# bowen-upenn/scene_graph_commonsense

Measured on AMD Instinct MI355X. Metric: ordered object-pairs/sec (relation head fwd+bwd), batch=8, N=64, higher is better.
Workload: dtype f16 fwd / bf16 bwd (f32 accumulate, f32 master weights); 1 GPU; VG PredCLS synthetic, 8 images x 64 objects per GPU = 32256 ordered pairs per GPU per step, from the raw minibatch; parallelism=dp1

## Files before the change

scene_graph_commonsense_amd/csrc/gemm_nt.h:

```cpp
#pragma once
#include "common.h"
#include <type_traits>

enum { AMODE_PLAIN = 0, AMODE_CONV = 1, AMODE_CONV_GATHER = 2 };
enum { EPI_STORE = 0, EPI_BIAS_TANH = 1, EPI_BIAS_RELU = 2, EPI_POOL = 3, EPI_FC2 = 4, EPI_RELUMASK = 5, EPI_STORE_F32 = 6,
       EPI_STORE_F32T = 7 };

struct NtParams {
    const u16* A; const u16* B; void* C;
    int M, N, K;
    long lda, ldb, ldc;
    int lgS, Cin;
    const float* bias;
    const u16* mask_src;
    const float* lsub; const float* lobj; const int* sub_idx; const int* obj_idx;
    unsigned char* argmax;
    u16* C2;
    float scale;
    unsigned drop_seed; int drop_enable;
    int tiles_m, tiles_n;
    int epi_lds;
    int halo_walk;
    int patch_aligned;
    const u16* Apool; const unsigned char* Acode;
    const int* gather; const int* gather_n;
    const int* dest;
    const int* wm_goff;
    float* raw; int raw_first;
    const int* tile_group; long group_stride;
    u16* Cx; int x_first;
    long seg_stride; int seg_bpad, seg_split;
};

template <int ELEM>
__device__ __forceinline__ f32x16 mfma32(s16x8 a, s16x8 b, f32x16 c) {
    if constexpr (ELEM == ELEM_F16) {
        return __builtin_amdgcn_mfma_f32_32x32x16_f16(__builtin_bit_cast(f16x8, a), __builtin_bit_cast(f16x8, b), c, 0, 0, 0);
    } else {
        return __builtin_amdgcn_mfma_f32_32x32x16_bf16(__builtin_bit_cast(bf16x8, a), __builtin_bit_cast(bf16x8, b), c, 0, 0, 0);
    }
}

__device__ __forceinline__ long conv_row_base(int m, int lgS, int Cin) {
    const int S = 1 << lgS;
    const int img = m >> (2 * lgS);
    const int ml = m & (S * S - 1);
    const int W = ml >> 2, q = ml & 3;
    const int py = W >> (lgS - 1), px = W & ((S >> 1) - 1);
    const int y = 2 * py + (q >> 1), x = 2 * px + (q & 1);
    return ((long)(img * (S + 2) + y) * (S + 2) + x) * Cin;
}

template <int ELEM, int EPI, int TM, int TN, bool GATHER = false>
__device__ __forceinline__ void nt_epilogue(const NtParams& p, f32x16 (&acc)[TM][TN], int m0, int n0, int wr, int wc, int lane, int m_limit = -1) {
    const int M = GATHER ? m_limit : p.M;
    const int h = lane >> 5, cl = lane & 31;
#pragma unroll
    for (int i = 0; i < TM; ++i) {
#pragma unroll
        for (int j = 0; j < TN; ++j) {
            const int col = n0 + wc * TN * 32 + j * 32 + cl;
            const int rbase = m0 + wr * TM * 32 + i * 32;
            const float bias = p.bias ? p.bias[col] : 0.f;
            if constexpr (EPI == EPI_POOL) {
                u16* out = reinterpret_cast<u16*>(p.C);
#pragma unroll
                for (int w = 0; w < 4; ++w) {
                    float v = acc[i][j][4 * w];
                    int am = 0;
#pragma unroll
                    for (int q = 1; q < 4; ++q) {
                        const float t = acc[i][j][4 * w + q];
                        if (t > v) { v = t; am = q; }
                    }
                    v += bias;
                    const int prow = (rbase >> 2) + 2 * w + h;
                    if (prow * 4 < M) {
                        long arow = prow, yrow = prow;
                        if constexpr (GATHER) {
                            arow = p.gather[prow]; yrow = p.dest ? p.dest[prow] : arow;
                            if (p.raw && prow >= p.raw_first) {
#pragma unroll
                                for (int q = 0; q < 4; ++q) p.raw[((long)(prow - p.raw_first) * 4 + q) * p.ldc + col] = acc[i][j][4 * w + q];
                            }
                        }
                        else if (p.wm_goff) yrow = p.wm_goff[prow & 63] + (prow >> 6);
                        if (!(v > 0.f)) { v = 0.f; am = 4; }
                        out[yrow * p.ldc + col] = to_elem<ELEM>(v);
                        if (p.C2) p.C2[yrow * p.ldc + col] = f32_to_bf16_bits(v);
                        if (p.argmax) p.argmax[arow * p.ldc + col] = (unsigned char)am;
                    }
                }
            } else {
#pragma unroll
                for (int r = 0; r < 16; ++r) {
                    const int row = rbase + (r & 3) + 8 * (r >> 2) + 4 * h;
                    if (row >= M) continue;
                    float v = acc[i][j][r];
                    long o = (long)row * p.ldc + col;
                    if constexpr (GATHER && EPI == EPI_STORE)
                        o = ((long)p.gather[row >> 2] * 4 + (row & 3)) * p.ldc + col;
                    if constexpr (EPI == EPI_STORE) {
                        reinterpret_cast<u16*>(p.C)[o] = to_elem<ELEM>(v + bias);
                    } else if constexpr (EPI == EPI_STORE_F32) {
                        reinterpret_cast<float*>(p.C)[o] = v + bias;
                    } else if constexpr (EPI == EPI_BIAS_TANH) {
                        reinterpret_cast<u16*>(p.C)[o] = to_elem<ELEM>(tanhf(v + bias));
                    } else if constexpr (EPI == EPI_BIAS_RELU) {
                        v = fmaxf(v + bias, 0.f);
                        if (p.drop_enable) v = dropout_keep(p.drop_seed, (uint32_t)(row * p.N + col)) ? v * p.scale : 0.f;
                        reinterpret_cast<u16*>(p.C)[o] = to_elem<ELEM>(v);
                    } else if constexpr (EPI == EPI_FC2) {
                        v += bias + p.lsub[(long)p.sub_idx[row] * p.N + col] + p.lobj[(long)p.obj_idx[row] * p.N + col];
                        v = fmaxf(v, 0.f);
                        if (p.drop_enable) v = dropout_keep(p.drop_seed, (uint32_t)(row * p.N + col)) ? v * p.scale : 0.f;
                        reinterpret_cast<float*>(p.C)[o] = v;
                    } else if constexpr (EPI == EPI_RELUMASK) {
                        const float f = from_elem<ELEM_F16>(p.mask_src[o]);
                        reinterpret_cast<u16*>(p.C)[o] = to_elem<ELEM>(f > 0.f ? v * p.scale : 0.f);
                    }
                }
            }
        }
    }
}

__device__ __forceinline__ void nt_epilogue_f32t(const NtParams& p, f32x16 (&acc)[4][2], int m0, int n0, int wr, int wc, int lane) {
    const int h = lane >> 5, cl = lane & 31;
    float* out = reinterpret_cast<float*>(p.C);
    if (!out) return;
    const int g_first = p.Cx ? p.wm_goff[p.tile_group[m0 >> 8]] + p.x_first : 0;
#pragma unroll
    for (int i = 0; i < 4; ++i) {
        const int row = m0 + wr * 128 + i * 32 + cl;
        if (row >= p.M) continue;
        const bool xrow = p.Cx && row >= g_first;
#pragma unroll
        for (int j = 0; j < 2; ++j) {
#pragma unroll
            for (int rq = 0; rq < 4; ++rq) {
                const int col = n0 + wc * 64 + j * 32 + 8 * rq + 4 * h;
                f32x4 v = {acc[i][j][4 * rq], acc[i][j][4 * rq + 1], acc[i][j][4 * rq + 2], acc[i][j][4 * rq + 3]};
                if (p.bias) {
                    const f32x4 b = *reinterpret_cast<const f32x4*>(p.bias + col);
                    v += b;
                }
                if (xrow) {
                    uint2 hv;
                    hv.x = (unsigned)f32_to_f16_bits(v[0]) | ((unsigned)f32_to_f16_bits(v[1]) << 16);
                    hv.y = (unsigned)f32_to_f16_bits(v[2]) | ((unsigned)f32_to_f16_bits(v[3]) << 16);
                    *reinterpret_cast<uint2*>(p.Cx + (long)row * p.N + col) = hv;
                    continue;
                }
                f32x4* dst = reinterpret_cast<f32x4*>(out + (long)row * p.ldc + col);
                *dst = v;
            }
        }
    }
}

__device__ __forceinline__ void supertile_map(int id, int tiles_m, int tiles_n, int& tm, int& tn) {
    constexpr int GS = 16;
    const int a = id / (GS * tiles_n);
    const int hm = min(GS, tiles_m - a * GS);
    const int id2 = id - a * GS * tiles_n;
    const int sn = (tiles_n + GS - 1) / GS;
    const int b = min(id2 / (hm * GS), sn - 1);
    const int id3 = id2 - b * hm * GS;
    const int wn = min(GS, tiles_n - b * GS);
    tm = a * GS + id3 / wn;
    tn = b * GS + id3 % wn;
}

__device__ __forceinline__ void supertile_map_g(int id, int tiles_m, int tiles_n, int GM, int GN, int& tm, int& tn) {
    const int a = id / (GM * tiles_n);
    const int hm = min(GM, tiles_m - a * GM);
    const int id2 = id - a * GM * tiles_n;
    const int sn = (tiles_n + GN - 1) / GN;
    const int b = min(id2 / (hm * GN), sn - 1);
    const int id3 = id2 - b * hm * GN;
    const int wn = min(GN, tiles_n - b * GN);
    tm = a * GM + id3 / wn;
    tn = b * GN + id3 % wn;
}

constexpr int EPI_LDS_PITCH = 128;
constexpr int EPI_LDS_BYTES = 8 * 128 * EPI_LDS_PITCH;
template <int ELEM, bool MASK = false>
__device__ __forceinline__ void nt_epilogue_store16(const NtParams& p, f32x16 (&acc)[4][2], int m0, int n0, int wr, int wc, int lane,
                                                    int wid, char* smem) {
    __syncthreads();
    char* reg = smem + wid * (128 * EPI_LDS_PITCH);
    const int h = lane >> 5, cl = lane & 31;
    const bool odd = cl & 1;
#pragma unroll
    for (int i = 0; i < 4; ++i) {
#pragma unroll
        for (int j = 0; j < 2; ++j) {
            const int col = n0 + wc * 64 + j * 32 + cl;
            const float bias = p.bias ? p.bias[col] : 0.f;
#pragma unroll
            for (int rp = 0; rp < 8; ++rp) {
                float v0 = acc[i][j][2 * rp] + bias, v1 = acc[i][j][2 * rp + 1] + bias;
                if constexpr (MASK) { v0 *= p.scale; v1 *= p.scale; }
                const float recv = __shfl_xor(odd ? v0 : v1, 1);
                const int r0 = ((2 * rp) & 3) + 8 * ((2 * rp) >> 2) + 4 * h;
                const float flo = odd ? recv : v0, fhi = odd ? v1 : recv;
                unsigned packed;
                if constexpr (ELEM == ELEM_BF16) packed = f32x2_to_bf16x2_bits(flo, fhi);
                else packed = (unsigned)to_elem<ELEM>(flo) | ((unsigned)to_elem<ELEM>(fhi) << 16);
                const int row = i * 32 + r0 + (odd ? 1 : 0);
                *reinterpret_cast<unsigned*>(reg + row * EPI_LDS_PITCH + (((j * 32 + (cl & ~1)) * 2) ^ ((row & 1) << 6))) = packed;
            }
        }
    }
    __builtin_amdgcn_wave_barrier();
    u16* out = reinterpret_cast<u16*>(p.C);
    const int c8 = lane & 7, rsub = lane >> 3;
#pragma unroll
    for (int it = 0; it < 16; ++it) {
        const int rowl = it * 8 + rsub;
        uint4 v = *reinterpret_cast<const uint4*>(reg + rowl * EPI_LDS_PITCH + ((c8 * 16) ^ ((rowl & 1) << 6)));
        const int row = m0 + wr * 128 + rowl;
        if (row < p.M) {
            const long o = (long)row * p.ldc + n0 + wc * 64 + c8 * 8;
            if constexpr (MASK) {
                const uint4 f = *reinterpret_cast<const uint4*>(p.mask_src + o);
                const u16* fh = reinterpret_cast<const u16*>(&f);
                u16* vh = reinterpret_cast<u16*>(&v);
#pragma unroll
                for (int k = 0; k < 8; ++k)
                    if (!(from_elem<ELEM_F16>(fh[k]) > 0.f)) vh[k] = 0;
            }
            *reinterpret_cast<uint4*>(out + o) = v;
        }
    }
}

template <int ELEM, int AMODE, int EPI, int WR, int WC, int TM, int TN>
__global__ __launch_bounds__(WR * WC * 64, 2) void gemm_nt_kernel(const NtParams p) {
    extern __shared__ __attribute__((aligned(16))) char smem[];
    constexpr int NW = WR * WC;
    constexpr int BM = WR * TM * 32, BN = WC * TN * 32;
    constexpr int A_BYTES = BM * 128, B_BYTES = BN * 128, BUF_BYTES = A_BYTES + B_BYTES;
    constexpr int AI = BM / (8 * NW), BI = BN / (8 * NW);
// ... 29 lines not shown
    const int Wp = (1 << p.lgS) + 2;

    auto stage = [&](int buf, int kt) {
        long aoff;
        if constexpr (AMODE != AMODE_PLAIN) {
            const int cc = kt / 9, tap = kt - cc * 9;
            const int ky = tap / 3, kx = tap - 3 * ky;
            aoff = (long)(ky * Wp + kx) * p.Cin + (cc << 6);
        } else {
            aoff = (long)kt << 6;
        }
        const long boff = (long)kt << 6;
        char* abase = smem + buf * BUF_BYTES + wid * (AI * 1024);
        char* bbase = smem + buf * BUF_BYTES + A_BYTES + wid * (BI * 1024);
#pragma unroll
        for (int i = 0; i < AI; ++i)
            __builtin_amdgcn_global_load_lds(GLB_PTR(a_ptr[i] + aoff), LDS_PTR(abase + i * 1024), 16, 0, 0);
#pragma unroll
        for (int i = 0; i < BI; ++i)
            __builtin_amdgcn_global_load_lds(GLB_PTR(b_ptr[i] + boff), LDS_PTR(bbase + i * 1024), 16, 0, 0);
    };

    const int wr = wid / WC, wc = wid % WC;
    const int kh = lane >> 5;
    int a_off[TM], a_sw[TM], b_off[TN], b_sw[TN];
#pragma unroll
    for (int i = 0; i < TM; ++i) {
        const int ra = wr * TM * 32 + i * 32 + (lane & 31);
        a_off[i] = ra * 128; a_sw[i] = (ra >> 1) & 7;
    }
#pragma unroll
    for (int i = 0; i < TN; ++i) {
        const int rb = wc * TN * 32 + i * 32 + (lane & 31);
        b_off[i] = rb * 128; b_sw[i] = (rb >> 1) & 7;
    }
    f32x16 acc[TM][TN];
#pragma unroll
    for (int i = 0; i < TM; ++i)
#pragma unroll
        for (int j = 0; j < TN; ++j)
#pragma unroll
            for (int r = 0; r < 16; ++r) acc[i][j][r] = 0.f;

    const int nk = p.K >> 6;
    stage(0, 0);
    for (int kt = 0; kt < nk; ++kt) {
        asm volatile("s_waitcnt vmcnt(0)" ::: "memory");
        __syncthreads();
        if (kt + 1 < nk) stage((kt + 1) & 1, kt + 1);
        const char* ab = smem + (kt & 1) * BUF_BYTES;
        const char* bb = ab + A_BYTES;
#pragma unroll
        for (int ks = 0; ks < 4; ++ks) {
            const int c = ks * 2 + kh;
            s16x8 af[TM], bf[TN];
#pragma unroll
            for (int i = 0; i < TM; ++i) af[i] = *reinterpret_cast<const s16x8*>(ab + a_off[i] + ((c ^ a_sw[i]) << 4));
#pragma unroll
            for (int i = 0; i < TN; ++i) bf[i] = *reinterpret_cast<const s16x8*>(bb + b_off[i] + ((c ^ b_sw[i]) << 4));
#pragma unroll
            for (int i = 0; i < TM; ++i)
#pragma unroll
                for (int j = 0; j < TN; ++j) acc[i][j] = mfma32<ELEM>(af[i], bf[j], acc[i][j]);
        }
    }

    if constexpr (EPI == EPI_STORE && TM == 4 && TN == 2 && WR * WC == 8) {
        if (p.epi_lds) { nt_epilogue_store16<ELEM>(p, acc, m0, n0, wr, wc, lane, wid, smem); return; }
    }
    if constexpr (AMODE == AMODE_CONV_GATHER) nt_epilogue<ELEM, EPI, TM, TN, true>(p, acc, m0, n0, wr, wc, lane, Mlim);
    else nt_epilogue<ELEM, EPI, TM, TN>(p, acc, m0, n0, wr, wc, lane);
}

template <int ELEM, int AMODE, int EPI, int WR, int WC, int TM, int TN>
static int launch_gemm_nt_cfg(NtParams p, hipStream_t stream) {
    constexpr int BM = WR * TM * 32, BN = WC * TN * 32;
    constexpr int LDS0 = 2 * (BM + BN) * 128;
    constexpr int LDS = (EPI == EPI_STORE && TM == 4 && TN == 2 && WR * WC == 8 && LDS0 < EPI_LDS_BYTES) ? EPI_LDS_BYTES : LDS0;
    p.tiles_m = (p.M + BM - 1) / BM;
    p.tiles_n = p.N / BN;
    auto kern = gemm_nt_kernel<ELEM, AMODE, EPI, WR, WC, TM, TN>;
    (void)hipFuncSetAttribute(reinterpret_cast<const void*>(kern), hipFuncAttributeMaxDynamicSharedMemorySize, LDS);
    SGC_LAUNCH(kern, dim3((unsigned)(p.tiles_m * p.tiles_n)), dim3(WR * WC * 64), LDS, stream, p);
    SGC_CHECK_LAUNCH();
    return SGC_OK;
}
// ... 22 lines not shown
```

scene_graph_commonsense_amd/csrc/gemm_nt_pp.h:

```cpp
#pragma once

#define SGC_WAIT_VM(n) asm volatile("s_waitcnt vmcnt(" #n ")" ::: "memory")
#define SGC_WAIT_LGKM0() asm volatile("s_waitcnt lgkmcnt(0)" ::: "memory")
#define SGC_PP_BARRIER()                                       \
    do {                                                       \
        __builtin_amdgcn_sched_barrier(0);                     \
        __builtin_amdgcn_s_barrier();                          \
        __builtin_amdgcn_sched_barrier(0);                     \
    } while (0)

__device__ __forceinline__ void buf_load_lds16(const void* base, int voff, int soff, void* lds) {
    const __amdgpu_buffer_rsrc_t r = __builtin_amdgcn_make_buffer_rsrc(const_cast<void*>(base), 0, 0x7fffffff, 0x00020000);
    __builtin_amdgcn_raw_ptr_buffer_load_lds(r, LDS_PTR(lds), 16, voff, soff, 0, 0);
}

__device__ __forceinline__ void xcd_patch_map(int id, int tiles_m, int tiles_n, int& tm, int& tn, int gm = 4, int gn = 8) {
    const int nb = tiles_m * tiles_n, q = nb >> 3, r = nb & 7, x = id & 7;
    const int lin = (x < r ? x * (q + 1) : r * (q + 1) + (x - r) * q) + (id >> 3);
    supertile_map_g(lin, tiles_m, tiles_n, gm, gn, tm, tn);
}

__host__ __device__ __forceinline__ int xcd_patch_gn(int tiles_n) { return tiles_n >= 8 ? 8 : (tiles_n >= 4 ? 4 : (tiles_n >= 2 ? 2 : 1)); }
static inline int xcd_patch_grid(int tiles_m, int tiles_n) {
    const int gn = xcd_patch_gn(tiles_n), gm = 32 / gn;
    const int npatch = ((tiles_m + gm - 1) / gm) * ((tiles_n + gn - 1) / gn);
    return ((npatch + 7) / 8) * 8 * 32;
}
__device__ __forceinline__ bool xcd_patch_map_aligned(int id, int tiles_m, int tiles_n, int& tm, int& tn) {
    const int gn = xcd_patch_gn(tiles_n), gm = 32 / gn;
    const int sn = (tiles_n + gn - 1) / gn, npatch = ((tiles_m + gm - 1) / gm) * sn;
    const int x = id & 7, j = id >> 3;
    const int patch = (j >> 5) * 8 + x, w = j & 31;
    if (patch >= npatch) return false;
    const int a = patch / sn, b = patch - a * sn;
    const int wn = min(gn, tiles_n - b * gn);
    tm = a * gm + w / wn;
    tn = b * gn + w % wn;
    return tm < tiles_m && w < gm * wn;
}

template <int ELEM, bool GATHER>
__device__ __forceinline__ void nt_epilogue_pool16(const NtParams& p, f32x16 (&acc)[4][2], int m0, int n0, int wr, int wc, int lane,
                                                   int wid, char* smem, int m_limit);
template <int ELEM, int EPI, int ACG = 0, int SEG = 0>
__global__ __launch_bounds__(512, 2) void gemm_nt_pp_kernel(const NtParams p) {
    extern __shared__ __attribute__((aligned(16))) char smem[];
    constexpr int HT = 16384;
    const int tid = threadIdx.x, lane = tid & 63;
    const int wid = __builtin_amdgcn_readfirstlane(tid >> 6);
    const int wr = wid >> 2, wc = wid & 3;
    int tm, tn;
    if constexpr (SEG) {
        xcd_patch_map(blockIdx.x, p.tiles_m, p.tiles_n, tm, tn, 16, 2);
    } else if (p.patch_aligned) {
        if (!xcd_patch_map_aligned(blockIdx.x, p.tiles_m, p.tiles_n, tm, tn)) return;
    } else {
        xcd_patch_map(blockIdx.x, p.tiles_m, p.tiles_n, tm, tn);
    }
    const int m0 = tm * 256;
    int n0 = tn * 256, n_tile = tn, Kloc = p.K, seg_py = 0, seg_px = 0, seg_ny = 1, seg_nx = 1, seg_c0 = 0;
    long ldb = p.ldb, b_off = 0;
    if constexpr (SEG) {
        const int slot = tn >> 1;
        int pp = 0, part = 0;
        if (p.seg_split) {
// ... 55 lines not shown
        char* base = smem + (((t & 1) << 2) + kind) * HT + wid * 2048;
        const u16* g = (kind == 0 || kind == 3) ? a_blk : b_blk;
        int soff = t << 7;
        if constexpr (ACG) {
            if (kind == 0 || kind == 3) {
                const int cc = t / 9, tap = t - cc * 9;
                const int ky = tap / 3, kx = tap - 3 * ky;
                soff = ((ky * SP + kx) * p.Cin + (cc << 6)) * 2;
            }
        }
        if constexpr (SEG) {
            if (kind == 0 || kind == 3) {
                const int c = seg_c0 + (t >> 4);
                const int cy = seg_nx == 2 ? (c >> 1) : c, cx = seg_nx == 2 ? (c & 1) : 0;
                const int qy = seg_ny == 1 ? (seg_py == 3) : cy, qx = seg_nx == 1 ? (seg_px == 3) : cx;
                g = a_blk + (long)(qy * 2 + qx) * p.seg_stride;
                soff = (t & 15) << 7;
            }
        }
        buf_load_lds16(g, voff[kind][0], soff, base);
        buf_load_lds16(g, voff[kind][1], soff, base + 1024);
    };

    const int l31 = lane & 31, kh = lane >> 5, sw = (l31 >> 1) & 7;
    int ko[4];
#pragma unroll
    for (int ks = 0; ks < 4; ++ks) ko[ks] = ((ks * 2 + kh) ^ sw) << 4;
    const int a_rd = (wr * 64 + l31) * 128, b_rd = (wc * 32 + l31) * 128;
    s16x8 af[2][4], bf[2][4];
    auto read_a = [&](int h, int par) __attribute__((always_inline)) {
        const char* base = smem + ((par << 2) + (h ? 3 : 0)) * HT + a_rd;
#pragma unroll
        for (int i = 0; i < 2; ++i)
#pragma unroll
            for (int ks = 0; ks < 4; ++ks) af[i][ks] = *reinterpret_cast<const s16x8*>(base + i * 4096 + ko[ks]);
    };
    auto read_b = [&](int par) __attribute__((always_inline)) {
#pragma unroll
        for (int h = 0; h < 2; ++h) {
            const char* base = smem + ((par << 2) + 1 + h) * HT + b_rd;
#pragma unroll
            for (int ks = 0; ks < 4; ++ks) bf[h][ks] = *reinterpret_cast<const s16x8*>(base + ko[ks]);
        }
    };

    f32x16 acc[4][2];
#pragma unroll
    for (int i = 0; i < 4; ++i)
#pragma unroll
        for (int j = 0; j < 2; ++j)
#pragma unroll
            for (int r = 0; r < 16; ++r) acc[i][j][r] = 0.f;
    auto half = [&](int a) __attribute__((always_inline)) {
        __builtin_amdgcn_sched_barrier(0);
#pragma unroll
        for (int ks = 0; ks < 4; ++ks)
#pragma unroll
            for (int i = 0; i < 2; ++i)
#pragma unroll
                for (int j = 0; j < 2; ++j) {
                    if constexpr (EPI == EPI_STORE_F32T) acc[2 * a + i][j] = mfma32<ELEM>(bf[j][ks], af[i][ks], acc[2 * a + i][j]);
                    else acc[2 * a + i][j] = mfma32<ELEM>(af[i][ks], bf[j][ks], acc[2 * a + i][j]);
                }
        SGC_PP_BARRIER();
    };
#define SGC_PP_CLOSE(STEADY)                                   \
    do {                                                       \
        if (STEADY) SGC_WAIT_VM(8); else SGC_WAIT_VM(0);       \
        SGC_WAIT_LGKM0();                                      \
        SGC_PP_BARRIER();                                      \
    } while (0)

    const int nk = Kloc >> 6;
    stage(0, 0); stage(1, 0); stage(2, 0); stage(3, 0);
    if (nk > 1) { stage(0, 1); stage(1, 1); stage(2, 1); SGC_WAIT_VM(8); } else SGC_WAIT_VM(0);
    __builtin_amdgcn_s_barrier();
    if (wr == 1) __builtin_amdgcn_s_barrier();

    auto tile = [&](int t, int par, auto steady_c) __attribute__((always_inline)) {
        constexpr bool STEADY = decltype(steady_c)::value;
        read_a(0, par); read_b(par);
        if (t + 1 < nk) stage(3, t + 1);
        SGC_PP_CLOSE(STEADY);
        half(0);
        read_a(1, par);
        if (STEADY) { stage(0, t + 2); stage(1, t + 2); stage(2, t + 2); }
        SGC_PP_CLOSE(STEADY);
        half(1);
    };
    int t = 0;
#pragma unroll 1
    for (; t + 2 < nk; ++t) tile(t, t & 1, std::true_type{});
#pragma unroll 1
    for (; t < nk; ++t) tile(t, t & 1, std::false_type{});
    if (wr == 0) __builtin_amdgcn_s_barrier();

    bool stored = false;
    if constexpr (EPI == EPI_STORE && !ACG) {
        if (p.epi_lds) { nt_epilogue_store16<ELEM>(p, acc, m0, n0, wr, wc, lane, wid, smem); stored = true; }
    }
    if constexpr (EPI == EPI_RELUMASK && !ACG) {
        if (p.epi_lds && !p.bias && (p.ldc & 7) == 0) { nt_epilogue_store16<ELEM, true>(p, acc, m0, n0, wr, wc, lane, wid, smem); stored = true; }
    }
    if (stored) {
    } else if constexpr (EPI == EPI_STORE_F32T) {
        static_assert(!ACG, "transposed f32 tile: plain rows only");
        nt_epilogue_f32t(p, acc, m0, n0, wr, wc, lane);
    }
    else if constexpr (ACG && EPI == EPI_POOL) {
        if (p.epi_lds) nt_epilogue_pool16<ELEM, true>(p, acc, m0, n0, wr, wc, lane, wid, smem, Mlim);
        else nt_epilogue<ELEM, EPI, 4, 2, true>(p, acc, m0, n0, wr, wc, lane, Mlim);
    }
    else if constexpr (ACG) nt_epilogue<ELEM, EPI, 4, 2, true>(p, acc, m0, n0, wr, wc, lane, Mlim);
    else nt_epilogue<ELEM, EPI, 4, 2>(p, acc, m0, n0, wr, wc, lane);
}

template <int ELEM, int EPI>
static int launch_gemm_nt_pp_conv_gather(NtParams p, hipStream_t stream) {
    constexpr int LDS = 8 * 16384;
    if ((p.lgS != 4 && p.lgS != 5) || (p.Cin & 63) || p.K != 9 * p.Cin || (p.N & 255)) return SGC_ERR_ARG;
    p.tiles_m = (p.M + 255) / 256;
    p.tiles_n = p.N / 256;
    p.patch_aligned = 0;
    if (EPI == EPI_POOL) p.epi_lds = 1;
    auto kern = gemm_nt_pp_kernel<ELEM, EPI, 1>;
    (void)hipFuncSetAttribute(reinterpret_cast<const void*>(kern), hipFuncAttributeMaxDynamicSharedMemorySize, LDS);
    SGC_LAUNCH(kern, dim3((unsigned)(p.tiles_m * p.tiles_n)), dim3(512), LDS, stream, p);
    SGC_CHECK_LAUNCH();
    return SGC_OK;
}
// ... 11 lines not shown
    SGC_CHECK_LAUNCH();
    return SGC_OK;
}

template <int ELEM, int EPI>
static int launch_gemm_nt_pp(NtParams p, hipStream_t stream) {
    constexpr int LDS = (EPI == EPI_STORE) ? EPI_LDS_BYTES : 8 * 16384;
    p.tiles_m = (p.M + 255) / 256;
    p.tiles_n = p.N / 256;
    auto kern = gemm_nt_pp_kernel<ELEM, EPI>;
    (void)hipFuncSetAttribute(reinterpret_cast<const void*>(kern), hipFuncAttributeMaxDynamicSharedMemorySize, LDS);
    const int grid_aligned = xcd_patch_grid(p.tiles_m, p.tiles_n);
    const int nb = p.tiles_m * p.tiles_n;
    p.patch_aligned = (nb >= 1024 && (nb & 255) != 0 && grid_aligned * 10 <= nb * 11) ? 1 : 0;
    SGC_LAUNCH(kern, dim3((unsigned)(p.patch_aligned ? grid_aligned : p.tiles_m * p.tiles_n)), dim3(512), LDS, stream, p);
    SGC_CHECK_LAUNCH();
    return SGC_OK;
}


constexpr int POOL_EPI_PY = 128, POOL_EPI_PA = 64;
constexpr int POOL_EPI_WAVE_BYTES = 32 * POOL_EPI_PY * 2 + 32 * POOL_EPI_PA;
template <int ELEM, bool GATHER>
__device__ __forceinline__ void nt_epilogue_pool16(const NtParams& p, f32x16 (&acc)[4][2], int m0, int n0, int wr, int wc, int lane,
                                                   int wid, char* smem, int m_limit) {
    __syncthreads();
    char* ty = smem + wid * POOL_EPI_WAVE_BYTES;
    char* tb = ty + 32 * POOL_EPI_PY;
    char* ta = tb + 32 * POOL_EPI_PY;
    const int h = lane >> 5, cl = lane & 31;
#pragma unroll
    for (int i = 0; i < 4; ++i)
#pragma unroll
        for (int j = 0; j < 2; ++j) {
            const int colw = j * 32 + cl;
            const float bias = p.bias ? p.bias[n0 + wc * 64 + colw] : 0.f;
#pragma unroll
            for (int w = 0; w < 4; ++w) {
                float v = acc[i][j][4 * w];
                int am = 0;
#pragma unroll
                for (int q = 1; q < 4; ++q) {
                    const float t = acc[i][j][4 * w + q];
                    if (t > v) { v = t; am = q; }
                }
                v += bias;
                if (!(v > 0.f)) { v = 0.f; am = 4; }
                const int row = i * 8 + 2 * w + h;
                if constexpr (GATHER) {
                    const int prow = (m0 >> 2) + wr * 32 + row;
                    if (p.raw && prow >= p.raw_first && prow * 4 < m_limit) {
#pragma unroll
                        for (int q = 0; q < 4; ++q) p.raw[((long)(prow - p.raw_first) * 4 + q) * p.ldc + n0 + wc * 64 + colw] = acc[i][j][4 * w + q];
                    }
                }
                *reinterpret_cast<u16*>(ty + row * POOL_EPI_PY + colw * 2) = to_elem<ELEM>(v);
                if (p.C2) *reinterpret_cast<u16*>(tb + row * POOL_EPI_PY + colw * 2) = f32_to_bf16_bits(v);
                if (p.argmax) *reinterpret_cast<unsigned char*>(ta + row * POOL_EPI_PA + colw) = (unsigned char)am;
            }
        }
    __builtin_amdgcn_wave_barrier();
    const long prow0 = ((long)m0 >> 2) + wr * 32;
    const int c8 = lane & 7, r8 = lane >> 3;
    u16* out = reinterpret_cast<u16*>(p.C);
#pragma unroll
    for (int it = 0; it < 4; ++it) {
        const int row = it * 8 + r8;
        long orow = prow0 + row;
        if constexpr (GATHER) {
            if (orow * 4 >= m_limit) continue;
            orow = p.dest ? p.dest[orow] : p.gather[orow];
        } else if (p.wm_goff) orow = p.wm_goff[orow & 63] + (orow >> 6);
        const long o = orow * p.ldc + n0 + wc * 64 + c8 * 8;
        *reinterpret_cast<uint4*>(out + o) = *reinterpret_cast<const uint4*>(ty + row * POOL_EPI_PY + c8 * 16);
        if (p.C2) *reinterpret_cast<uint4*>(p.C2 + o) = *reinterpret_cast<const uint4*>(tb + row * POOL_EPI_PY + c8 * 16);
    }
    if (p.argmax) {
        const int c4 = lane & 3, r16 = lane >> 2;
#pragma unroll
        for (int it = 0; it < 2; ++it) {
            const int row = it * 16 + r16;
            long arow = prow0 + row;
            if constexpr (GATHER) {
                if (arow * 4 >= m_limit) continue;
                arow = p.gather[arow];
            }
            *reinterpret_cast<uint4*>(p.argmax + arow * p.ldc + n0 + wc * 64 + c4 * 16) =
                *reinterpret_cast<const uint4*>(ta + row * POOL_EPI_PA + c4 * 16);
        }
    }
}

template <int ELEM, int EPI, int ASRC = 0>
__global__ __launch_bounds__(512, 2) void conv16_halo_pp_kernel(const NtParams p) {
    extern __shared__ __attribute__((aligned(16))) char smem[];
    constexpr int A_BYTES = 328 * 128;
    constexpr int HT = 16384;
    char* const abuf0 = smem;
    char* const bbuf0 = smem + 2 * A_BYTES;
    const int tid = threadIdx.x, lane = tid & 63;
    const int wid = __builtin_amdgcn_readfirstlane(tid >> 6);
    const int wr = wid >> 2, wc = wid & 3;
    int img, tn;
    if (p.halo_walk) {
        const int nb = p.tiles_m * p.tiles_n, q = nb >> 3, r = nb & 7, x = blockIdx.x & 7;
        const int lin = (x < r ? x * (q + 1) : r * (q + 1) + (x - r) * q) + (blockIdx.x >> 3);
        img = lin / p.tiles_n; tn = lin - img * p.tiles_n;
    } else {
        img = blockIdx.x / p.tiles_n; tn = blockIdx.x - img * p.tiles_n;
    }
    const int m0 = img * 256, n0 = tn * 256;
    const int Cin = p.Cin;

    const int lrow = lane >> 3, cpos = lane & 7;
    int a_off[6];
#pragma unroll
    for (int i = 0; i < 6; ++i) {
        int r = (wid + 8 * i) * 8 + lrow;
        if (r > 323) r = 323;
        const int py = r / 18, px = r - py * 18;
        const int f = ((px >> 1) + 4 * (py & 1)) & 7;
        a_off[i] = r * Cin + ((cpos ^ f) << 3);
    }
    const u16* const a_img = ASRC ? p.A : p.A + (long)img * (324L * Cin);
    const int npiece = ASRC ? 0 : ((wid == 0) ? 6 : 5);
    auto stage_a_piece = [&](int i, int cc) __attribute__((always_inline)) {
        buf_load_lds16(a_img, a_off[i] * 2, cc << 7, abuf0 + (cc & 1) * A_BYTES + (wid + 8 * i) * 1024);
    };
    char* const pscr = smem + 2 * A_BYTES + 4 * HT;
    const int pw = tid >> 3, pg = tid & 7;
    const u16* const apool_img = ASRC ? p.Apool + (long)img * 64 * Cin : nullptr;
    const unsigned char* const acode_img = ASRC ? p.Acode + (long)img * 64 * Cin : nullptr;
    const int pool_voff = (pw * Cin + pg * 8) * 2;
    const int pool_coff = (wid * 16 + (lane >> 2)) * Cin + (lane & 3) * 16;
    const int npool = (wid < 4) ? 2 : 1;
    auto pool_dma = [&](int cc) __attribute__((always_inline)) {
        buf_load_lds16(apool_img, pool_voff, cc << 7, pscr + wid * 1024);
        if (wid < 4) buf_load_lds16(acode_img, pool_coff, cc << 6, pscr + 8192 + wid * 1024);
    };
    auto pool_scatter_q = [&](int cc, int q) __attribute__((always_inline)) {
        char* ab = abuf0 + (cc & 1) * A_BYTES;
        const uint4 pool_v = *reinterpret_cast<const uint4*>(pscr + tid * 16);
        const uint2 pool_c = *reinterpret_cast<const uint2*>(pscr + 8192 + pw * 64 + pg * 8);
        const u16* vh = reinterpret_cast<const u16*>(&pool_v);
        const unsigned char* ch = reinterpret_cast<const unsigned char*>(&pool_c);
        const int wy = pw >> 3, wx = pw & 7;
        const unsigned qq = (unsigned)q * 0x01010101u;
        const unsigned x0 = pool_c.x ^ qq, x1 = pool_c.y ^ qq;
        const unsigned m0 = ~(((x0 & 0x7f7f7f7fu) + 0x7f7f7f7fu) | x0) & 0x80808080u;
        const unsigned m1 = ~(((x1 & 0x7f7f7f7fu) + 0x7f7f7f7fu) | x1) & 0x80808080u;
        auto lanes = [](unsigned m, int e) __attribute__((always_inline)) {
            const unsigned lo = (unsigned)__builtin_amdgcn_sbfe(m, 8 * e + 7, 1), hi = (unsigned)__builtin_amdgcn_sbfe(m, 8 * e + 15, 1);
            return (lo & 0x0000ffffu) | (hi & 0xffff0000u);
        };
        uint4 o;
        o.x = pool_v.x & lanes(m0, 0); o.y = pool_v.y & lanes(m0, 2); o.z = pool_v.z & lanes(m1, 0); o.w = pool_v.w & lanes(m1, 2);
        (void)vh; (void)ch;
        const int py = 2 * wy + (q >> 1) + 1, px = 2 * wx + (q & 1) + 1;
        const int f = ((px >> 1) + 4 * (py & 1)) & 7;
        *reinterpret_cast<uint4*>(ab + (py * 18 + px) * 128 + ((pg ^ f) << 4)) = o;
    };
    auto pool_scatter = [&](int cc) __attribute__((always_inline)) {
#pragma unroll
        for (int q = 0; q < 4; ++q) pool_scatter_q(cc, q);
    };
    const u16* const b_blk = p.B + (long)n0 * p.ldb;
    int b_voff[2][2];
#pragma unroll
    for (int q = 0; q < 2; ++q) {
        const int r = (wid * 2 + q) * 8 + lrow;
        const int chunk = (cpos ^ ((r >> 1) & 7)) << 3;
#pragma unroll
        for (int h = 0; h < 2; ++h) b_voff[h][q] = (int)((((r >> 5) * 64 + h * 32 + (r & 31)) * p.ldb + chunk) * 2);
    }
    auto stage_b = [&](int step) __attribute__((always_inline)) {
        char* base = bbuf0 + ((step & 1) * 2) * HT + wid * 2048;
#pragma unroll
        for (int h = 0; h < 2; ++h) {
            buf_load_lds16(b_blk, b_voff[h][0], step << 7, base + h * HT);
            buf_load_lds16(b_blk, b_voff[h][1], step << 7, base + h * HT + 1024);
        }
    };

    const int l31 = lane & 31, kh = lane >> 5;
    int a_row[4], a_px[4], a_py[4];
#pragma unroll
    for (int i = 0; i < 4; ++i) {
        const int m = wr * 128 + i * 32 + l31;
        const int W = m >> 2, q = m & 3;
        a_py[i] = 2 * (W >> 3) + (q >> 1);
        a_px[i] = 2 * (W & 7) + (q & 1);
        a_row[i] = a_py[i] * 18 + a_px[i];
    }
    const int bsw = (l31 >> 1) & 7;
    int bko[4];
#pragma unroll
    for (int ks = 0; ks < 4; ++ks) bko[ks] = ((ks * 2 + kh) ^ bsw) << 4;
    const int b_rd = (wc * 32 + l31) * 128;
    s16x8 af[2][4], bf[2][4];
    auto read_a = [&](int h, int cc, int ky, int kx) __attribute__((always_inline)) {
        const char* ab = abuf0 + (cc & 1) * A_BYTES;
#pragma unroll
        for (int i = 0; i < 2; ++i) {
            const int ii = 2 * h + i;
            const char* rowp = ab + (a_row[ii] + ky * 18 + kx) * 128;
            const int f = (((a_px[ii] + kx) >> 1) + 4 * ((a_py[ii] + ky) & 1)) & 7;
#pragma unroll
            for (int ks = 0; ks < 4; ++ks) af[i][ks] = *reinterpret_cast<const s16x8*>(rowp + (((ks * 2 + kh) ^ f) << 4));
        }
    };
    auto read_b = [&](int step) __attribute__((always_inline)) {
#pragma unroll
        for (int h = 0; h < 2; ++h) {
            const char* base = bbuf0 + ((step & 1) * 2 + h) * HT + b_rd;
#pragma unroll
            for (int ks = 0; ks < 4; ++ks) bf[h][ks] = *reinterpret_cast<const s16x8*>(base + bko[ks]);
        }
    };

    f32x16 acc[4][2];
#pragma unroll
    for (int i = 0; i < 4; ++i)
#pragma unroll
        for (int j = 0; j < 2; ++j)
#pragma unroll
            for (int r = 0; r < 16; ++r) acc[i][j][r] = 0.f;
    auto half = [&](int a) __attribute__((always_inline)) {
        __builtin_amdgcn_sched_barrier(0);
#pragma unroll
        for (int ks = 0; ks < 4; ++ks)
#pragma unroll
            for (int i = 0; i < 2; ++i)
#pragma unroll
                for (int j = 0; j < 2; ++j) acc[2 * a + i][j] = mfma32<ELEM>(af[i][ks], bf[j][ks], acc[2 * a + i][j]);
        SGC_PP_BARRIER();
    };

    const int ncc = Cin >> 6;
    const int nsteps = ncc * 9;
    if constexpr (ASRC) {
        pool_dma(0);
        for (int i = tid; i < 2 * A_BYTES / 16; i += 512)
            *reinterpret_cast<uint4*>(abuf0 + i * 16) = make_uint4(0, 0, 0, 0);
        SGC_WAIT_VM(0);
        __syncthreads();
        pool_scatter(0);
        stage_b(0);
        if (nsteps > 1) { stage_b(1); SGC_WAIT_VM(4); } else SGC_WAIT_VM(0);
        SGC_WAIT_LGKM0();
    } else {
#pragma unroll
        for (int i = 0; i < 6; ++i)
            if (i < npiece) stage_a_piece(i, 0);
        stage_b(0);
        if (nsteps > 1) { stage_b(1); SGC_WAIT_VM(4); } else SGC_WAIT_VM(0);
    }
    __builtin_amdgcn_s_barrier();
// ... 79 lines not shown
```

Baseline: 855,300 pairs/s.

## Switch f16 GEMM and conv kernels to 16x16x32 MFMA with remapped fragments

```diff
diff --git a/scene_graph_commonsense_amd/csrc/gemm_nt.h b/scene_graph_commonsense_amd/csrc/gemm_nt.h
--- a/scene_graph_commonsense_amd/csrc/gemm_nt.h
+++ b/scene_graph_commonsense_amd/csrc/gemm_nt.h
@@ -41,6 +41,47 @@
     }
 }
 
+template <int ELEM>
+__device__ __forceinline__ f32x4 mfma16(s16x8 a, s16x8 b, f32x4 c) {
+    static_assert(ELEM == ELEM_F16, "the bf16 blocks stay on 32x32x16 (tied bit for bit to the sparse kernels)");
+    return __builtin_amdgcn_mfma_f32_16x16x32_f16(__builtin_bit_cast(f16x8, a), __builtin_bit_cast(f16x8, b), c, 0, 0, 0);
+}
+
+struct NtAcc16 {
+    f32x4 q[4];
+    __device__ __forceinline__ float operator[](int r) const { return q[r >> 2][r & 3]; }
+};
+template <int ELEM> struct nt_acc { typedef f32x16 type; };
+template <> struct nt_acc<ELEM_F16> { typedef NtAcc16 type; };
+template <int ELEM> using nt_acc_t = typename nt_acc<ELEM>::type;
+__device__ __forceinline__ void nt_acc_zero(f32x16& a) {
+#pragma unroll
+    for (int r = 0; r < 16; ++r) a[r] = 0.f;
+}
+__device__ __forceinline__ void nt_acc_zero(NtAcc16& a) {
+#pragma unroll
+    for (int w = 0; w < 4; ++w) a.q[w] = f32x4{0.f, 0.f, 0.f, 0.f};
+}
+template <int ELEM> __device__ __forceinline__ int quad_row(int w, int lane) {
+    if constexpr (ELEM == ELEM_F16) return 16 * (w >> 1) + 4 * (lane >> 4); else return 8 * w + 4 * (lane >> 5);
+}
+template <int ELEM> __device__ __forceinline__ int quad_col(int w, int lane) {
+    if constexpr (ELEM == ELEM_F16) return 16 * (w & 1) + (lane & 15); else return lane & 31;
+}
+template <int ELEM> __device__ __forceinline__ int frag_row(int lane) { return ELEM == ELEM_F16 ? (lane & 15) : (lane & 31); }
+template <int ELEM> __device__ __forceinline__ int frag_kh(int lane) { return ELEM == ELEM_F16 ? (lane >> 4) : (lane >> 5); }
+template <int ELEM, bool SWAP = false>
+__device__ __forceinline__ void mfma16_step(NtAcc16& acc, s16x8 a0, s16x8 a1, s16x8 b0, s16x8 b1) {
+#pragma unroll
+    for (int sa = 0; sa < 2; ++sa)
+#pragma unroll
+        for (int sb = 0; sb < 2; ++sb) {
+            const s16x8 a = sa ? a1 : a0, b = sb ? b1 : b0;
+            if constexpr (SWAP) acc.q[2 * sa + sb] = mfma16<ELEM>(b, a, acc.q[2 * sa + sb]);
+            else acc.q[2 * sa + sb] = mfma16<ELEM>(a, b, acc.q[2 * sa + sb]);
+        }
+}
+
 __device__ __forceinline__ long conv_row_base(int m, int lgS, int Cin) {
     const int S = 1 << lgS;
     const int img = m >> (2 * lgS);
@@ -52,20 +93,22 @@
 }
 
 template <int ELEM, int EPI, int TM, int TN, bool GATHER = false>
-__device__ __forceinline__ void nt_epilogue(const NtParams& p, f32x16 (&acc)[TM][TN], int m0, int n0, int wr, int wc, int lane, int m_limit = -1) {
+__device__ __forceinline__ void nt_epilogue(const NtParams& p, nt_acc_t<ELEM> (&acc)[TM][TN], int m0, int n0, int wr, int wc, int lane, int m_limit = -1) {
     const int M = GATHER ? m_limit : p.M;
-    const int h = lane >> 5, cl = lane & 31;
 #pragma unroll
     for (int i = 0; i < TM; ++i) {
 #pragma unroll
         for (int j = 0; j < TN; ++j) {
-            const int col = n0 + wc * TN * 32 + j * 32 + cl;
             const int rbase = m0 + wr * TM * 32 + i * 32;
-            const float bias = p.bias ? p.bias[col] : 0.f;
+            const float bias0 = p.bias ? p.bias[n0 + wc * TN * 32 + j * 32 + quad_col<ELEM>(0, lane)] : 0.f;
+            float bias1 = bias0;
+            if constexpr (ELEM == ELEM_F16) bias1 = p.bias ? p.bias[n0 + wc * TN * 32 + j * 32 + quad_col<ELEM>(1, lane)] : 0.f;
             if constexpr (EPI == EPI_POOL) {
                 u16* out = reinterpret_cast<u16*>(p.C);
 #pragma unroll
                 for (int w = 0; w < 4; ++w) {
+                    const int col = n0 + wc * TN * 32 + j * 32 + quad_col<ELEM>(w, lane);
+                    const float bias = (w & 1) ? bias1 : bias0;
                     float v = acc[i][j][4 * w];
                     int am = 0;
 #pragma unroll
@@ -74,7 +117,7 @@
                         if (t > v) { v = t; am = q; }
                     }
                     v += bias;
-                    const int prow = (rbase >> 2) + 2 * w + h;
+                    const int prow = (rbase + quad_row<ELEM>(w, lane)) >> 2;
                     if (prow * 4 < M) {
                         long arow = prow, yrow = prow;
                         if constexpr (GATHER) {
@@ -94,8 +137,10 @@
             } else {
 #pragma unroll
                 for (int r = 0; r < 16; ++r) {
-                    const int row = rbase + (r & 3) + 8 * (r >> 2) + 4 * h;
+                    const int row = rbase + quad_row<ELEM>(r >> 2, lane) + (r & 3);
                     if (row >= M) continue;
+                    const int col = n0 + wc * TN * 32 + j * 32 + quad_col<ELEM>(r >> 2, lane);
+                    const float bias = ((r >> 2) & 1) ? bias1 : bias0;
                     float v = acc[i][j][r];
                     long o = (long)row * p.ldc + col;
                     if constexpr (GATHER && EPI == EPI_STORE)
@@ -125,21 +170,23 @@
     }
 }
 
-__device__ __forceinline__ void nt_epilogue_f32t(const NtParams& p, f32x16 (&acc)[4][2], int m0, int n0, int wr, int wc, int lane) {
-    const int h = lane >> 5, cl = lane & 31;
+template <int ELEM>
+__device__ __forceinline__ void nt_epilogue_f32t(const NtParams& p, nt_acc_t<ELEM> (&acc)[4][2], int m0, int n0, int wr, int wc, int lane) {
     float* out = reinterpret_cast<float*>(p.C);
     if (!out) return;
     const int g_first = p.Cx ? p.wm_goff[p.tile_group[m0 >> 8]] + p.x_first : 0;
 #pragma unroll
     for (int i = 0; i < 4; ++i) {
-        const int row = m0 + wr * 128 + i * 32 + cl;
-        if (row >= p.M) continue;
-        const bool xrow = p.Cx && row >= g_first;
 #pragma unroll
         for (int j = 0; j < 2; ++j) {
 #pragma unroll
             for (int rq = 0; rq < 4; ++rq) {
-                const int col = n0 + wc * 64 + j * 32 + 8 * rq + 4 * h;
+                const int rloc = ELEM == ELEM_F16 ? 16 * (rq >> 1) + (lane & 15) : (lane & 31);
+                const int cloc = ELEM == ELEM_F16 ? 16 * (rq & 1) + 4 * (lane >> 4) : 8 * rq + 4 * (lane >> 5);
+                const int row = m0 + wr * 128 + i * 32 + rloc;
+                if (row >= p.M) continue;
+                const bool xrow = p.Cx && row >= g_first;
+                const int col = n0 + wc * 64 + j * 32 + cloc;
                 f32x4 v = {acc[i][j][4 * rq], acc[i][j][4 * rq + 1], acc[i][j][4 * rq + 2], acc[i][j][4 * rq + 3]};
                 if (p.bias) {
                     const f32x4 b = *reinterpret_cast<const f32x4*>(p.bias + col);
@@ -186,31 +233,37 @@
 
 constexpr int EPI_LDS_PITCH = 128;
 constexpr int EPI_LDS_BYTES = 8 * 128 * EPI_LDS_PITCH;
+template <int ELEM> __device__ __forceinline__ int epi_lds_key(int row) {
+    if constexpr (ELEM == ELEM_F16) return (((row ^ (row >> 3)) & 1) << 6) | (((row >> 2) & 1) << 5);
+    else return (row & 1) << 6;
+}
 template <int ELEM, bool MASK = false>
-__device__ __forceinline__ void nt_epilogue_store16(const NtParams& p, f32x16 (&acc)[4][2], int m0, int n0, int wr, int wc, int lane,
+__device__ __forceinline__ void nt_epilogue_store16(const NtParams& p, nt_acc_t<ELEM> (&acc)[4][2], int m0, int n0, int wr, int wc, int lane,
                                                     int wid, char* smem) {
     __syncthreads();
     char* reg = smem + wid * (128 * EPI_LDS_PITCH);
-    const int h = lane >> 5, cl = lane & 31;
-    const bool odd = cl & 1;
+    const bool odd = lane & 1;
 #pragma unroll
     for (int i = 0; i < 4; ++i) {
 #pragma unroll
         for (int j = 0; j < 2; ++j) {
-            const int col = n0 + wc * 64 + j * 32 + cl;
-            const float bias = p.bias ? p.bias[col] : 0.f;
+            const float bias0 = p.bias ? p.bias[n0 + wc * 64 + j * 32 + quad_col<ELEM>(0, lane)] : 0.f;
+            float bias1 = bias0;
+            if constexpr (ELEM == ELEM_F16) bias1 = p.bias ? p.bias[n0 + wc * 64 + j * 32 + quad_col<ELEM>(1, lane)] : 0.f;
 #pragma unroll
             for (int rp = 0; rp < 8; ++rp) {
+                const int cl = quad_col<ELEM>(rp >> 1, lane);
+                const float bias = ((rp >> 1) & 1) ? bias1 : bias0;
                 float v0 = acc[i][j][2 * rp] + bias, v1 = acc[i][j][2 * rp + 1] + bias;
                 if constexpr (MASK) { v0 *= p.scale; v1 *= p.scale; }
                 const float recv = __shfl_xor(odd ? v0 : v1, 1);
-                const int r0 = ((2 * rp) & 3) + 8 * ((2 * rp) >> 2) + 4 * h;
+                const int r0 = ((2 * rp) & 3) + quad_row<ELEM>(rp >> 1, lane);
                 const float flo = odd ? recv : v0, fhi = odd ? v1 : recv;
                 unsigned packed;
                 if constexpr (ELEM == ELEM_BF16) packed = f32x2_to_bf16x2_bits(flo, fhi);
                 else packed = (unsigned)to_elem<ELEM>(flo) | ((unsigned)to_elem<ELEM>(fhi) << 16);
                 const int row = i * 32 + r0 + (odd ? 1 : 0);
-                *reinterpret_cast<unsigned*>(reg + row * EPI_LDS_PITCH + (((j * 32 + (cl & ~1)) * 2) ^ ((row & 1) << 6))) = packed;
+                *reinterpret_cast<unsigned*>(reg + row * EPI_LDS_PITCH + (((j * 32 + (cl & ~1)) * 2) ^ epi_lds_key<ELEM>(row))) = packed;
             }
         }
     }
@@ -220,7 +273,7 @@
 #pragma unroll
     for (int it = 0; it < 16; ++it) {
         const int rowl = it * 8 + rsub;
-        uint4 v = *reinterpret_cast<const uint4*>(reg + rowl * EPI_LDS_PITCH + ((c8 * 16) ^ ((rowl & 1) << 6)));
+        uint4 v = *reinterpret_cast<const uint4*>(reg + rowl * EPI_LDS_PITCH + ((c8 * 16) ^ epi_lds_key<ELEM>(rowl)));
         const int row = m0 + wr * 128 + rowl;
         if (row < p.M) {
             const long o = (long)row * p.ldc + n0 + wc * 64 + c8 * 8;
@@ -296,25 +349,23 @@
     };
 
     const int wr = wid / WC, wc = wid % WC;
-    const int kh = lane >> 5;
+    const int kh = frag_kh<ELEM>(lane);
     int a_off[TM], a_sw[TM], b_off[TN], b_sw[TN];
 #pragma unroll
     for (int i = 0; i < TM; ++i) {
-        const int ra = wr * TM * 32 + i * 32 + (lane & 31);
+        const int ra = wr * TM * 32 + i * 32 + frag_row<ELEM>(lane);
         a_off[i] = ra * 128; a_sw[i] = (ra >> 1) & 7;
     }
 #pragma unroll
     for (int i = 0; i < TN; ++i) {
-        const int rb = wc * TN * 32 + i * 32 + (lane & 31);
+        const int rb = wc * TN * 32 + i * 32 + frag_row<ELEM>(lane);
         b_off[i] = rb * 128; b_sw[i] = (rb >> 1) & 7;
     }
-    f32x16 acc[TM][TN];
+    nt_acc_t<ELEM> acc[TM][TN];
 #pragma unroll
     for (int i = 0; i < TM; ++i)
 #pragma unroll
-        for (int j = 0; j < TN; ++j)
-#pragma unroll
-            for (int r = 0; r < 16; ++r) acc[i][j][r] = 0.f;
+        for (int j = 0; j < TN; ++j) nt_acc_zero(acc[i][j]);
 
     const int nk = p.K >> 6;
     stage(0, 0);
@@ -324,18 +375,38 @@
         if (kt + 1 < nk) stage((kt + 1) & 1, kt + 1);
         const char* ab = smem + (kt & 1) * BUF_BYTES;
         const char* bb = ab + A_BYTES;
-#pragma unroll
-        for (int ks = 0; ks < 4; ++ks) {
-            const int c = ks * 2 + kh;
-            s16x8 af[TM], bf[TN];
-#pragma unroll
-            for (int i = 0; i < TM; ++i) af[i] = *reinterpret_cast<const s16x8*>(ab + a_off[i] + ((c ^ a_sw[i]) << 4));
-#pragma unroll
-            for (int i = 0; i < TN; ++i) bf[i] = *reinterpret_cast<const s16x8*>(bb + b_off[i] + ((c ^ b_sw[i]) << 4));
-#pragma unroll
-            for (int i = 0; i < TM; ++i)
-#pragma unroll
-                for (int j = 0; j < TN; ++j) acc[i][j] = mfma32<ELEM>(af[i], bf[j], acc[i][j]);
+        if constexpr (ELEM == ELEM_F16) {
+#pragma unroll
+            for (int ks2 = 0; ks2 < 2; ++ks2) {
+                const int c = ks2 * 4 + kh;
+                s16x8 af[TM][2], bf[TN][2];
+#pragma unroll
+                for (int i = 0; i < TM; ++i)
+#pragma unroll
+                    for (int s = 0; s < 2; ++s) af[i][s] = *reinterpret_cast<const s16x8*>(ab + a_off[i] + s * 2048 + ((c ^ a_sw[i]) << 4));
+#pragma unroll
+                for (int i = 0; i < TN; ++i)
+#pragma unroll
+                    for (int s = 0; s < 2; ++s) bf[i][s] = *reinterpret_cast<const s16x8*>(bb + b_off[i] + s * 2048 + ((c ^ b_sw[i]) << 4));
+#pragma unroll
+                for (int i = 0; i < TM; ++i)
+#pragma unroll
+                    for (int j = 0; j < TN; ++j) mfma16_step<ELEM>(acc[i][j], af[i][0], af[i][1], bf[j][0], bf[j][1]);
+            }
+        } else {
+#pragma unroll
+            for (int ks = 0; ks < 4; ++ks) {
+                const int c = ks * 2 + kh;
+                s16x8 af[TM], bf[TN];
+#pragma unroll
+                for (int i = 0; i < TM; ++i) af[i] = *reinterpret_cast<const s16x8*>(ab + a_off[i] + ((c ^ a_sw[i]) << 4));
+#pragma unroll
+                for (int i = 0; i < TN; ++i) bf[i] = *reinterpret_cast<const s16x8*>(bb + b_off[i] + ((c ^ b_sw[i]) << 4));
+#pragma unroll
+                for (int i = 0; i < TM; ++i)
+#pragma unroll
+                    for (int j = 0; j < TN; ++j) acc[i][j] = mfma32<ELEM>(af[i], bf[j], acc[i][j]);
+            }
         }
     }
 
diff --git a/scene_graph_commonsense_amd/csrc/gemm_nt_pp.h b/scene_graph_commonsense_amd/csrc/gemm_nt_pp.h
--- a/scene_graph_commonsense_amd/csrc/gemm_nt_pp.h
+++ b/scene_graph_commonsense_amd/csrc/gemm_nt_pp.h
@@ -40,7 +40,7 @@
 }
 
 template <int ELEM, bool GATHER>
-__device__ __forceinline__ void nt_epilogue_pool16(const NtParams& p, f32x16 (&acc)[4][2], int m0, int n0, int wr, int wc, int lane,
+__device__ __forceinline__ void nt_epilogue_pool16(const NtParams& p, nt_acc_t<ELEM> (&acc)[4][2], int m0, int n0, int wr, int wc, int lane,
                                                    int wid, char* smem, int m_limit);
 template <int ELEM, int EPI, int ACG = 0, int SEG = 0>
 __global__ __launch_bounds__(512, 2) void gemm_nt_pp_kernel(const NtParams p) {
@@ -142,11 +142,12 @@
         buf_load_lds16(g, voff[kind][1], soff, base + 1024);
     };
 
-    const int l31 = lane & 31, kh = lane >> 5, sw = (l31 >> 1) & 7;
+    constexpr bool M16 = ELEM == ELEM_F16;
+    const int lr = frag_row<ELEM>(lane), kh = frag_kh<ELEM>(lane), sw = (lr >> 1) & 7;
     int ko[4];
 #pragma unroll
-    for (int ks = 0; ks < 4; ++ks) ko[ks] = ((ks * 2 + kh) ^ sw) << 4;
-    const int a_rd = (wr * 64 + l31) * 128, b_rd = (wc * 32 + l31) * 128;
+    for (int f = 0; f < 4; ++f) ko[f] = M16 ? (f >> 1) * 2048 + ((((f & 1) * 4 + kh) ^ sw) << 4) : ((f * 2 + kh) ^ sw) << 4;
+    const int a_rd = (wr * 64 + lr) * 128, b_rd = (wc * 32 + lr) * 128;
     s16x8 af[2][4], bf[2][4];
     auto read_a = [&](int h, int par) __attribute__((always_inline)) {
         const char* base = smem + ((par << 2) + (h ? 3 : 0)) * HT + a_rd;
@@ -164,24 +165,32 @@
         }
     };
 
-    f32x16 acc[4][2];
+    nt_acc_t<ELEM> acc[4][2];
 #pragma unroll
     for (int i = 0; i < 4; ++i)
 #pragma unroll
-        for (int j = 0; j < 2; ++j)
-#pragma unroll
-            for (int r = 0; r < 16; ++r) acc[i][j][r] = 0.f;
+        for (int j = 0; j < 2; ++j) nt_acc_zero(acc[i][j]);
     auto half = [&](int a) __attribute__((always_inline)) {
         __builtin_amdgcn_sched_barrier(0);
-#pragma unroll
-        for (int ks = 0; ks < 4; ++ks)
-#pragma unroll
-            for (int i = 0; i < 2; ++i)
-#pragma unroll
-                for (int j = 0; j < 2; ++j) {
-                    if constexpr (EPI == EPI_STORE_F32T) acc[2 * a + i][j] = mfma32<ELEM>(bf[j][ks], af[i][ks], acc[2 * a + i][j]);
-                    else acc[2 * a + i][j] = mfma32<ELEM>(af[i][ks], bf[j][ks], acc[2 * a + i][j]);
-                }
+        if constexpr (M16) {
+#pragma unroll
+            for (int ks2 = 0; ks2 < 2; ++ks2)
+#pragma unroll
+                for (int i = 0; i < 2; ++i)
+#pragma unroll
+                    for (int j = 0; j < 2; ++j)
+                        mfma16_step<ELEM, EPI == EPI_STORE_F32T>(acc[2 * a + i][j], af[i][ks2], af[i][2 + ks2], bf[j][ks2], bf[j][2 + ks2]);
+        } else {
+#pragma unroll
+            for (int ks = 0; ks < 4; ++ks)
+#pragma unroll
+                for (int i = 0; i < 2; ++i)
+#pragma unroll
+                    for (int j = 0; j < 2; ++j) {
+                        if constexpr (EPI == EPI_STORE_F32T) acc[2 * a + i][j] = mfma32<ELEM>(bf[j][ks], af[i][ks], acc[2 * a + i][j]);
+                        else acc[2 * a + i][j] = mfma32<ELEM>(af[i][ks], bf[j][ks], acc[2 * a + i][j]);
+                    }
+        }
         SGC_PP_BARRIER();
     };
 #define SGC_PP_CLOSE(STEADY)                                   \
@@ -225,7 +234,7 @@
     if (stored) {
     } else if constexpr (EPI == EPI_STORE_F32T) {
         static_assert(!ACG, "transposed f32 tile: plain rows only");
-        nt_epilogue_f32t(p, acc, m0, n0, wr, wc, lane);
+        nt_epilogue_f32t<ELEM>(p, acc, m0, n0, wr, wc, lane);
     }
     else if constexpr (ACG && EPI == EPI_POOL) {
         if (p.epi_lds) nt_epilogue_pool16<ELEM, true>(p, acc, m0, n0, wr, wc, lane, wid, smem, Mlim);
@@ -283,21 +292,20 @@
 constexpr int POOL_EPI_PY = 128, POOL_EPI_PA = 64;
 constexpr int POOL_EPI_WAVE_BYTES = 32 * POOL_EPI_PY * 2 + 32 * POOL_EPI_PA;
 template <int ELEM, bool GATHER>
-__device__ __forceinline__ void nt_epilogue_pool16(const NtParams& p, f32x16 (&acc)[4][2], int m0, int n0, int wr, int wc, int lane,
+__device__ __forceinline__ void nt_epilogue_pool16(const NtParams& p, nt_acc_t<ELEM> (&acc)[4][2], int m0, int n0, int wr, int wc, int lane,
                                                    int wid, char* smem, int m_limit) {
     __syncthreads();
     char* ty = smem + wid * POOL_EPI_WAVE_BYTES;
     char* tb = ty + 32 * POOL_EPI_PY;
     char* ta = tb + 32 * POOL_EPI_PY;
-    const int h = lane >> 5, cl = lane & 31;
 #pragma unroll
     for (int i = 0; i < 4; ++i)
 #pragma unroll
         for (int j = 0; j < 2; ++j) {
-            const int colw = j * 32 + cl;
-            const float bias = p.bias ? p.bias[n0 + wc * 64 + colw] : 0.f;
 #pragma unroll
             for (int w = 0; w < 4; ++w) {
+                const int colw = j * 32 + quad_col<ELEM>(w, lane);
+                const float bias = p.bias ? p.bias[n0 + wc * 64 + colw] : 0.f;
                 float v = acc[i][j][4 * w];
                 int am = 0;
 #pragma unroll
@@ -307,7 +315,7 @@
                 }
                 v += bias;
                 if (!(v > 0.f)) { v = 0.f; am = 4; }
-                const int row = i * 8 + 2 * w + h;
+                const int row = i * 8 + (quad_row<ELEM>(w, lane) >> 2);
                 if constexpr (GATHER) {
                     const int prow = (m0 >> 2) + wr * 32 + row;
                     if (p.raw && prow >= p.raw_first && prow * 4 < m_limit) {
@@ -352,6 +360,9 @@
     }
 }
 
+template <int ELEM> __device__ __forceinline__ int halo_swz(int py, int px) {
+    if constexpr (ELEM == ELEM_F16) return (2 * (px >> 1) + (py & 1)) & 7; else return ((px >> 1) + 4 * (py & 1)) & 7;
+}
 template <int ELEM, int EPI, int ASRC = 0>
 __global__ __launch_bounds__(512, 2) void conv16_halo_pp_kernel(const NtParams p) {
     extern __shared__ __attribute__((aligned(16))) char smem[];
@@ -380,7 +391,7 @@
         int r = (wid + 8 * i) * 8 + lrow;
         if (r > 323) r = 323;
         const int py = r / 18, px = r - py * 18;
-        const int f = ((px >> 1) + 4 * (py & 1)) & 7;
+        const int f = halo_swz<ELEM>(py, px);
         a_off[i] = r * Cin + ((cpos ^ f) << 3);
     }
     const u16* const a_img = ASRC ? p.A : p.A + (long)img * (324L * Cin);
@@ -418,7 +429,7 @@
         o.x = pool_v.x & lanes(m0, 0); o.y = pool_v.y & lanes(m0, 2); o.z = pool_v.z & lanes(m1, 0); o.w = pool_v.w & lanes(m1, 2);
         (void)vh; (void)ch;
         const int py = 2 * wy + (q >> 1) + 1, px = 2 * wx + (q & 1) + 1;
-        const int f = ((px >> 1) + 4 * (py & 1)) & 7;
+        const int f = halo_swz<ELEM>(py, px);
         *reinterpret_cast<uint4*>(ab + (py * 18 + px) * 128 + ((pg ^ f) << 4)) = o;
     };
     auto pool_scatter = [&](int cc) __attribute__((always_inline)) {
@@ -443,21 +454,22 @@
         }
     };
 
-    const int l31 = lane & 31, kh = lane >> 5;
+    constexpr bool M16 = ELEM == ELEM_F16;
+    const int lr = frag_row<ELEM>(lane), kh = frag_kh<ELEM>(lane);
     int a_row[4], a_px[4], a_py[4];
 #pragma unroll
     for (int i = 0; i < 4; ++i) {
-        const int m = wr * 128 + i * 32 + l31;
+        const int m = wr * 128 + i * 32 + lr;
         const int W = m >> 2, q = m & 3;
         a_py[i] = 2 * (W >> 3) + (q >> 1);
         a_px[i] = 2 * (W & 7) + (q & 1);
         a_row[i] = a_py[i] * 18 + a_px[i];
     }
-    const int bsw = (l31 >> 1) & 7;
+    const int bsw = (lr >> 1) & 7;
     int bko[4];
 #pragma unroll
-    for (int ks = 0; ks < 4; ++ks) bko[ks] = ((ks * 2 + kh) ^ bsw) << 4;
-    const int b_rd = (wc * 32 + l31) * 128;
+    for (int f = 0; f < 4; ++f) bko[f] = M16 ? (f >> 1) * 2048 + ((((f & 1) * 4 + kh) ^ bsw) << 4) : ((f * 2 + kh) ^ bsw) << 4;
+    const int b_rd = (wc * 32 + lr) * 128;
     s16x8 af[2][4], bf[2][4];
     auto read_a = [&](int h, int cc, int ky, int kx) __attribute__((always_inline)) {
         const char* ab = abuf0 + (cc & 1) * A_BYTES;
@@ -465,9 +477,12 @@
         for (int i = 0; i < 2; ++i) {
             const int ii = 2 * h + i;
             const char* rowp = ab + (a_row[ii] + ky * 18 + kx) * 128;
-            const int f = (((a_px[ii] + kx) >> 1) + 4 * ((a_py[ii] + ky) & 1)) & 7;
-#pragma unroll
-            for (int ks = 0; ks < 4; ++ks) af[i][ks] = *reinterpret_cast<const s16x8*>(rowp + (((ks * 2 + kh) ^ f) << 4));
+            const int f = halo_swz<ELEM>(a_py[ii] + ky, a_px[ii] + kx);
+#pragma unroll
+            for (int ks = 0; ks < 4; ++ks) {
+                if constexpr (M16) af[i][ks] = *reinterpret_cast<const s16x8*>(rowp + (ks >> 1) * 1024 + ((((ks & 1) * 4 + kh) ^ f) << 4));
+                else af[i][ks] = *reinterpret_cast<const s16x8*>(rowp + (((ks * 2 + kh) ^ f) << 4));
+            }
         }
     };
     auto read_b = [&](int step) __attribute__((always_inline)) {
@@ -479,21 +494,29 @@
         }
     };
 
-    f32x16 acc[4][2];
+    nt_acc_t<ELEM> acc[4][2];
 #pragma unroll
     for (int i = 0; i < 4; ++i)
 #pragma unroll
-        for (int j = 0; j < 2; ++j)
-#pragma unroll
-            for (int r = 0; r < 16; ++r) acc[i][j][r] = 0.f;
+        for (int j = 0; j < 2; ++j) nt_acc_zero(acc[i][j]);
     auto half = [&](int a) __attribute__((always_inline)) {
         __builtin_amdgcn_sched_barrier(0);
-#pragma unroll
-        for (int ks = 0; ks < 4; ++ks)
-#pragma unroll
-            for (int i = 0; i < 2; ++i)
-#pragma unroll
-                for (int j = 0; j < 2; ++j) acc[2 * a + i][j] = mfma32<ELEM>(af[i][ks], bf[j][ks], acc[2 * a + i][j]);
+        if constexpr (M16) {
+#pragma unroll
+            for (int ks2 = 0; ks2 < 2; ++ks2)
+#pragma unroll
+                for (int i = 0; i < 2; ++i)
+#pragma unroll
+                    for (int j = 0; j < 2; ++j)
+                        mfma16_step<ELEM>(acc[2 * a + i][j], af[i][ks2], af[i][2 + ks2], bf[j][ks2], bf[j][2 + ks2]);
+        } else {
+#pragma unroll
+            for (int ks = 0; ks < 4; ++ks)
+#pragma unroll
+                for (int i = 0; i < 2; ++i)
+#pragma unroll
+                    for (int j = 0; j < 2; ++j) acc[2 * a + i][j] = mfma32<ELEM>(af[i][ks], bf[j][ks], acc[2 * a + i][j]);
+        }
         SGC_PP_BARRIER();
     };
 
```

New measurement: 793,700 pairs/s. 0.928x the previous value.
